# tzmhuang/OmniIsaacGymEnvs

Hardware: AMD Instinct MI355X
Metric: env-steps/s (physics+obs+reward) Humanoid 4096 envs @1/2/4/8 MI355X (higher is better)
Workload: dtype f32

## Files before the change

### include/mi_sim.h

```cpp
#ifndef MI_SIM_H
#define MI_SIM_H

#include <stdint.h>

#ifdef __cplusplus
extern "C" {
#endif

#define MI_ABI_VERSION 4

enum {
    MI_OK = 0,
    MI_E_NULL = -1,
    MI_E_SHAPE = -2,
    MI_E_HIP = -3,
    MI_E_MODEL = -4,
    MI_E_ARG = -5,
    MI_E_NODEV = -6,
    MI_E_STATE = -7
};

enum { MI_TASK_CARTPOLE = 0, MI_TASK_ANT = 1, MI_TASK_HUMANOID = 2 };

enum {
// ... 58 lines not shown
    int32_t num_obs;
    int32_t num_actions;
    float clip_actions, clip_obs;
    float max_episode_length;
    float power_scale, heading_weight, up_weight, actions_cost, energy_cost;
    float dof_vel_scale, angular_velocity_scale, contact_force_scale;
    float joints_at_limit_cost, death_cost, termination_height, alive_reward_scale;
    float task_dt;
    float target[3];
    float init_root_pos[3];
    float init_root_quat[4];
    float dof_pos_noise, dof_vel_noise;
    const float* joint_gears;
    const float* motor_effort_ratio;
    const float* init_dof_pos;
    float reset_dist, max_push_effort;
} mi_task_params;

#define MI_MAX_ROWS 128

typedef struct mi_sim mi_sim;

int mi_sim_create(const mi_model_desc* model, const mi_sim_params* params, int32_t num_envs,
                  int64_t env_id_offset, int32_t device_id, const float* env_origins ,
                  uint64_t seed, mi_sim** out);
int mi_sim_destroy(mi_sim* sim);
int mi_sim_info(const mi_sim* sim, int32_t* num_envs, int32_t* num_dof, int32_t* num_links,
                int32_t* num_sensors, float* dof_limits );

int mi_get_root_state(mi_sim* sim, float* pos , float* quat ,
                      float* vel , void* stream);
int mi_get_dof_state(mi_sim* sim, float* q , float* qd , void* stream);
int mi_get_sensor_wrench(mi_sim* sim, float* out , void* stream);
int mi_set_dof_efforts(mi_sim* sim, const float* eff , const int32_t* idx ,
                       int32_t n, void* stream);
int mi_set_dof_state(mi_sim* sim, const float* q , const float* qd ,
                     const int64_t* idx , int32_t n, void* stream);
int mi_set_root_state(mi_sim* sim, const float* pos , const float* quat ,
                      const float* vel , const int64_t* idx , int32_t n,
                      void* stream);
int mi_set_dof_state_i32(mi_sim* sim, const float* q , const float* qd ,
                         const int32_t* idx , int32_t n, void* stream);
int mi_set_root_state_i32(mi_sim* sim, const float* pos , const float* quat ,
                          const float* vel , const int32_t* idx , int32_t n,
                          void* stream);
int mi_get_link_state(mi_sim* sim, const int32_t* link_ids , const float* offsets ,
                      int32_t K, float* pos, float* quat, float* vel, void* stream);
int mi_get_link_jacobian(mi_sim* sim, const int32_t* link_ids, const float* offsets, int32_t K,
                         float* jac, void* stream);
int mi_get_dynamics(mi_sim* sim, float* M, float* cor, float* grav, void* stream);
enum { MI_MASS_ARMATURE = 0,
       MI_MASS_STEPPER  = 1 };

int mi_solve_mass(mi_sim* sim, int32_t which, const float* rhs, int32_t R, float* out, void* stream);

int mi_get_forward_dynamics(mi_sim* sim, int32_t which, const float* tau, float* acc, void* stream);

int mi_get_link_task_inertia(mi_sim* sim, int32_t which, const int32_t* link_ids, const float* offsets,
                             int32_t K, float* minv_jt, float* lam_inv, void* stream);
enum { MI_MASS_RIGID = 2 };

int mi_get_inverse_dynamics(mi_sim* sim, int32_t which, const float* acc, float* tau, float* joint_wrench,
                            void* stream);

int mi_get_link_acceleration(mi_sim* sim, const int32_t* link_ids, const float* offsets, int32_t K,
                             const float* acc, float* out, void* stream);

int mi_get_momentum(mi_sim* sim, float* com, float* mom, float* cmm, float* energy, void* stream);
int mi_sim_set_mirror(mi_sim* sim, float* pos , float* quat , float* vel ,
                      float* q , float* qd , float* sens );
int mi_get_state_mirror(mi_sim* sim, void* stream);

int mi_sim_step(mi_sim* sim, int32_t substeps, void* stream);
int mi_sim_flush(mi_sim* sim, void* stream);

int mi_task_configure(mi_sim* sim, const mi_task_params* tp);
int mi_task_pre_step(mi_sim* sim, const float* actions , int64_t* reset_buf,
                     int64_t* progress_buf, float* potentials, float* prev_potentials,
                     float* actions_out , void* stream);
int mi_task_reset_idx(mi_sim* sim, const int64_t* env_ids, int32_t n, int64_t* reset_buf,
                      int64_t* progress_buf, float* potentials, float* prev_potentials,
                      void* stream);
int mi_task_post_step(mi_sim* sim, const float* actions , float* obs ,
                      float* rew , int64_t* reset_buf, int64_t* progress_buf,
                      float* potentials, float* prev_potentials, void* stream);
int mi_task_post_kernel(const mi_sim* sim, int32_t* kernel, int32_t* grid);
int mi_task_observations(mi_sim* sim, const float* actions , float* obs ,
                         float* potentials, float* prev_potentials, void* stream);
int mi_task_metrics(mi_sim* sim, const float* actions, const float* obs, float* rew,
                    const float* potentials, const float* prev_potentials, void* stream);
int mi_task_is_done(mi_sim* sim, const float* obs, int64_t* reset_buf, const int64_t* progress_buf,
                    void* stream);
int mi_env_step(mi_sim* sim, const float* actions , int32_t substeps,
                float* obs_out , float* obs_task ,
                float* rew , int64_t* reset_buf, int64_t* progress_buf,
                float* potentials, float* prev_potentials, float* actions_out ,
                float* rew_out , int64_t* reset_out , void* stream);
int mi_sim_time_launches(mi_sim* sim, int32_t every, int32_t capacity);
int mi_sim_launch_times(mi_sim* sim, float* ms_out, int32_t max_out, int32_t* n_out);

enum { MI_DR_OP_ADDITIVE = 0, MI_DR_OP_SCALING = 1 };
enum { MI_DR_DIST_GAUSSIAN = 0, MI_DR_DIST_UNIFORM = 1, MI_DR_DIST_LOGUNIFORM = 2 };
typedef struct mi_dr_noise {
    int32_t enabled;
    int32_t operation;
    int32_t distribution;
    int32_t frequency_interval;
    float params[2];
} mi_dr_noise;
typedef struct mi_dr_params {
    mi_dr_noise obs_on_reset, obs_on_interval, act_on_reset, act_on_interval;
} mi_dr_params;
int mi_task_set_dr(mi_sim* sim, const mi_dr_params* dr );
int mi_dr_apply_actions(mi_sim* sim, float* actions , const int64_t* reset_buf, void* stream);
int mi_dr_apply_observations(mi_sim* sim, float* obs , const int64_t* reset_buf,
                             void* stream);
int mi_get_dr_state(mi_sim* sim, uint32_t* out );

enum { MI_ENVP_GRAVITY = 0,
       MI_ENVP_FRICTION = 1,
       MI_ENVP_DAMPING = 2,
       MI_ENVP_ARMATURE = 3    };
int mi_set_env_params(mi_sim* sim, int32_t attr, const float* values ,
                      const int64_t* idx , int32_t n, void* stream);
int mi_get_env_params(mi_sim* sim, int32_t attr, float* out , void* stream);
int mi_sim_clear_env_params(mi_sim* sim);

enum { MI_DR_OP_DIRECT = 2 };
typedef struct mi_dr_phys_sched {
    int32_t enabled;
    int32_t operation;
    int32_t distribution;
    int32_t frequency_interval;
    const float* p0;
    const float* p1;
} mi_dr_phys_sched;
typedef struct mi_dr_phys_params {
    mi_dr_phys_sched on_reset[4], on_interval[4];
    int32_t min_frequency;
} mi_dr_phys_params;
int mi_sim_set_phys_dr(mi_sim* sim, const mi_dr_phys_params* dr );
int mi_dr_phys_step(mi_sim* sim, const int64_t* reset_buf , void* stream);
int mi_get_phys_dr_state(mi_sim* sim, uint32_t* out );

int mi_fill_uniform(mi_sim* sim, float* out , int32_t cols, uint64_t seed,
                    uint64_t step, float lo, float hi, void* stream);
int mi_get_reset_count(mi_sim* sim, uint32_t* out );
int mi_set_reset_count(mi_sim* sim, const uint32_t* in );
int mi_sim_pair_load(mi_sim* sim, int32_t* out , const int32_t* in ,
                     int32_t pairing);
int mi_sim_nan_count(mi_sim* sim, int64_t* count);
int mi_sim_kernel_path(const mi_sim* sim, int32_t* path, int32_t* topology, int32_t* lds_bytes);
int mi_sim_w_rows_lds(const mi_sim* sim, int32_t* rows);
int mi_abi_version(void);
const char* mi_build_id(void);
const char* mi_last_error(void);

#ifdef __cplusplus
}
#endif
#endif
```

### omniisaacgymenvs_amd/csrc/mi_pair.hpp

```cpp
#pragma once
#include "mi_wave.hpp"

#ifndef MI_PAIR_SOLVE_PD
#define MI_PAIR_SOLVE_PD 3
#endif
#ifndef MI_PRIO_C1
#define MI_PRIO_C1 12
#endif
#ifndef MI_PRIO_C2
#define MI_PRIO_C2 18
#endif
#ifndef MI_PRIO_C3
#define MI_PRIO_C3 27
#endif

namespace mi {

MI_D float pbc(float v, int k) {
    const float a = readlane(v, k), b = readlane(v, k + 32);
    return (pair_l64() & 32) ? b : a;
}
template <int K>
MI_D float pbcc(float v) {
    static_assert(K >= 0 && K < 32, "lane of the half");
// ... 17 lines not shown
        const int c = __popc((m >> b) & ((1u << w) - 1u));
        if (j >= c) { j -= c; b += w; }
    }
    return b;
}
MI_D unsigned low_bits(unsigned m, int k) {
    return k >= __popc(m) ? m : (m & ((1u << nth_bit(m, k)) - 1u));
}
MI_D int pmax(int v) { return max(__builtin_amdgcn_readlane(v, 0), __builtin_amdgcn_readlane(v, 32)); }
MI_D float psum(float v) { return pbc(half_sums(v), 31); }

template <class T>
MI_D float ct_ltdl_pair(int lane, float (&Mc)[T::nvc]) {
    float dvec = 1.0f;
    sfor_down<0, T::nv>([&](auto K) {
        constexpr int k = K;
        const int ln = lane_here(lane);
        const float inv = __builtin_amdgcn_rcpf(pbcc<k>(Mc[k]));
        const float t = Mc[k] * inv;
        sfor<T::dof.anc_start[k], T::dof.anc_start[k + 1]>([&](auto A) {
            constexpr int ii = T::dof.anc[A];
            Mc[ii] -= pbcc<ii>(t) * Mc[k];
        });
        Mc[k] = t;
        dvec = ln == k ? inv : dvec;
    });
    return dvec;
}

#ifndef MI_PAIR_WIDE_PD
#define MI_PAIR_WIDE_PD 16
#endif
#ifndef MI_PAIR_WIDE_AREG
#define MI_PAIR_WIDE_AREG 28
#endif
constexpr int kWideScratchRows = 64 - MI_PAIR_WIDE_AREG;
#ifndef MI_PAIR_WIDE_AP
#define MI_PAIR_WIDE_AP 8
#endif
#ifndef MI_PAIR_LIM_NEAR
#define MI_PAIR_LIM_NEAR 0.05f
#endif
#ifndef MI_PAIR_LIM_SPEC_MIN_D
#define MI_PAIR_LIM_SPEC_MIN_D 16
#endif
#ifndef MI_PAIR_JREUSE_MAXNV
#define MI_PAIR_JREUSE_MAXNV 16
#endif
typedef float pv2 __attribute__((ext_vector_type(2)));
template <int NV, int NVC>
MI_D float pk_jdot(const float (&J)[NVC], const float* u) {
    float v = 0.0f;
    sfor<0, NV>([&](auto C) { v += J[C] * u[C]; });
    return v;
}

template <class TP>
MI_D void pair_jrow(const MC& mc, const WaveTabs& t, const float* sm, int r, int nr,
                    float (&J)[TP::nvc]) {
    const float lk = sm[t.s_rl + r];
    float f[6] = {0.0f, 0.0f, 0.0f, 0.0f, 0.0f, 0.0f};
    unsigned msk = 0u, msk2 = 0u;
    float sg = 0.0f;
    int kdof = -1;
    if (lk >= 0.0f) {
        msk = mc.mask((int)lk);
        const float l2 = TP::kSelf ? sm[t.s_cl2 + r / 3] : -1.0f;
        msk2 = l2 >= 0.0f ? mc.mask((int)l2) : 0u;
        contact_row_f<TP::kSelf>(sm, t, r, f);
    } else {
        kdof = (int)(-lk - 1.0f);
        sg = sm[t.s_lsg + kdof - nr];
    }
    const float* Ss = sm + t.s_S;
    sdof_loop<TP, MI_PAIR_SDOF_PD, false, sdof_first_loaded(TP::nr)>(Ss, nullptr, [&](auto C, const float (&sv)[6], float) {
        constexpr int c = C;
        const float v = sdot<TP, c>(sv, f);
        const bool ia = (msk >> c) & 1u, ib = (msk2 >> c) & 1u;
        float xc = (ia ? v : 0.0f) - (ib ? v : 0.0f);
        asm volatile("" : "+v"(xc));
        J[c] = kdof >= 0 ? (kdof == c ? sg : 0.0f) : xc;
    });
}

typedef const float __attribute__((address_space(3)))* lds_cf;
MI_D lds_cf lds_ptr(const float* p) { return (lds_cf)p; }
typedef float pv4 __attribute__((ext_vector_type(4)));
typedef const pv4 __attribute__((address_space(3)))* lds_cf4;
MI_D int pw_idx(int r, int c, int nv) { return (r & ~3) * nv + 4 * c + (r & 3); }
MI_D size_t pair_sidx(int r, int c) { return (size_t)(r & ~3) * WNV + 4 * c + (r & 3); }
typedef const float __attribute__((address_space(1)))* glb_cf;
typedef float __attribute__((address_space(1)))* glb_f;
typedef const pv4 __attribute__((address_space(1)))* glb_cf4;
MI_D glb_cf glb_ptr(const float* p) { return (glb_cf)p; }
MI_D glb_f glb_ptr(float* p) { return (glb_f)p; }

struct WSrc {
    lds_cf W;
    glb_cf gW;
    int nl;
};
MI_D WSrc make_wsrc(const WaveTabs& t, const float* sm, glb_cf gW) {
    WSrc w;
    w.W = lds_ptr(sm + t.s_W);
    int nl = t.w_rows_lds;
    asm volatile("" : "+s"(nl));
    w.nl = nl;
    w.gW = gW;
    return w;
}

template <class TP, int PD, bool kLds>
MI_D void pair_dgroup_w(const WSrc& ws, int g0, int n, const float (&Jr)[TP::nvc], float (&a)[4]) {
    constexpr int NV = TP::nv, NB = PD + 1;
    pv2 a01 = {0.0f, 0.0f}, a23 = {0.0f, 0.0f};
    auto acc = [&](auto C, const pv4& w) {
        const pv2 j = {Jr[C], Jr[C]};
        a01 = __builtin_elementwise_fma(j, w.xy, a01);
        a23 = __builtin_elementwise_fma(j, w.zw, a23);
    };
    if (kLds || g0 + 3 < ws.nl) {
        const lds_cf4 W = (lds_cf4)(ws.W + g0 * NV);
        pv4 wb[NB];
        sfor<0, (PD < NV ? PD : NV)>([&](auto C) { wb[C % NB] = W[C]; });
        sfor<0, NV>([&](auto C) {
            constexpr int c = C;
            if constexpr (c + PD < NV) wb[(c + PD) % NB] = W[c + PD];
            acc(C, wb[c % NB]);
        });
    } else {
        const glb_cf4 W = (glb_cf4)(ws.gW + (size_t)g0 * WNV);
        pv4 wb[NB];
        sfor<0, (PD < NV ? PD : NV)>([&](auto C) { wb[C % NB] = W[C]; });
        sfor<0, NV>([&](auto C) {
            constexpr int c = C;
            if constexpr (c + PD < NV) wb[(c + PD) % NB] = W[c + PD];
            acc(C, wb[c % NB]);
        });
    }
    const float a0 = a01.x, a1 = a01.y, a2 = a23.x, a3 = a23.y;
    a[0] = g0 < n ? a0 : 0.0f;
    a[1] = g0 + 1 < n ? a1 : 0.0f;
    a[2] = g0 + 2 < n ? a2 : 0.0f;
    a[3] = g0 + 3 < n ? a3 : 0.0f;
}
template <bool kLds>
MI_D void pair_wcol_w(const WSrc& ws, int g0, int kc, int nv, float (&wq)[4]) {
    const pv4 w = (kLds || g0 + 3 < ws.nl) ? ((lds_cf4)(ws.W + g0 * nv))[kc]
                                           : ((glb_cf4)(ws.gW + (size_t)g0 * WNV))[kc];
    wq[0] = w.x; wq[1] = w.y; wq[2] = w.z; wq[3] = w.w;
}


template <class TP>
MI_D void pair_artic_substep(const DevModel& m, const WaveTabs& t, const DevState& st,
                             const SimP& p, int i, int wv_, const float* mcb, float* sm, float* gW_,
                             bool load_state, bool store_state, int& prio, int& load,
                             const float* ep = nullptr) {
    const glb_f gW = glb_ptr(gW_);
    static_assert(TP::kCT && TP::nv <= 32, "paired kernel: compiled topology, nv <= 32");
    const int lane = pair_l64() & 31;
    const int L = m.L, D = m.D, nv = m.nv, nr = m.nr;
    const float dt = p.dt;
    float* us = sm + t.s_us;
    float* rhs = sm + t.s_r;
    float* Mx = sm + t.s_M;
    float* Ss = sm + t.s_S;
    const MC mc = make_mc(t, mcb, L);

    STAMP_BEGIN();
    if (load_state) {
        if (lane < 3) sm[t.s_rp + lane] = st.root_pos[sx(st, lane, i)];
        if (lane < 4) sm[t.s_rp + 4 + lane] = st.root_quat[sx(st, lane, i)];
        if (lane < nr) us[lane] = st.root_vel[sx(st, lane, i)];
        else if (lane < nv) us[lane] = st.qd[sx(st, lane - nr, i)];
        if (lane < D) sm[t.s_q + lane] = st.q[sx(st, lane, i)];
    }
    if (nr && lane < 6) {
        float s[6] = {0, 0, 0, 0, 0, 0};
        if (lane < 3) s[3 + lane] = 1.0f; else s[lane - 3] = 1.0f;
#pragma unroll
        for (int c = 0; c < 6; ++c) Ss[6 * lane + c] = s[c];
    }
    wave_sync();
    STAMP(0);
    for (int l = 1 + lane; l < L; l += 32) wave_link_local(mc, t, sm, l);
    wave_sync();
    for (int l = lane; l < L; l += 32) wave_link_forward<TP::kEnvP>(mc, nr, t, sm, l, p, ep);
    wave_sync();
    STAMP(1);
    float* aux = sm + t.s_X;
    {
        const pv4* recs = reinterpret_cast<const pv4*>(sm + t.s_F);
        for (int l = lane; l < L; l += 32) {
            pv4 a0 = recs[4 * l], a1 = recs[4 * l + 1], a2 = recs[4 * l + 2], a3 = recs[4 * l + 3];
            for (int di = mc.desc_start(l); di < mc.desc_start(l + 1); ++di) {
                const int d = mc.desc(di);
                a0 += recs[4 * d];
                a1 += recs[4 * d + 1];
                a2 += recs[4 * d + 2];
                a3 += recs[4 * d + 3];
            }
            pv4* o = reinterpret_cast<pv4*>(aux) + 4 * l;
            o[0] = a0; o[1] = a1; o[2] = a2; o[3] = a3;
        }
    }
    wave_sync();
    STAMP(2);
    phase_p3_bias_crba<Grp32, TP>(lane, i, D, nv, nr, dt, us, rhs, Mx, Ss, mc, t, st, aux, ep);
    wave_sync();
    STAMP(3);
    float Mc[TP::nvc];
    ct_load_columns<TP>(Mx, lane, Mc);
    const float dvec = ct_ltdl_pair<TP>(lane, Mc);
    STAMP(5);
    {
        const int dj = lane < nr ? lane : __builtin_popcount(mc.mask(lane < nv ? lane - nr + 1 : 0)) - 1;
        ct_publish_factor<TP>(lane, dj, Mc, dvec, sm + t.s_L);
    }
    STAMP(4);
    int ncon = 0;
    {
        const float rpz = sm[t.s_rp + 2];
        for (int c0 = 0; c0 < t.npts; c0 += 32) {
            const int c = c0 + lane;
            bool act = false;
            float pc[3] = {0, 0, 0}, bn = 0.0f;
            int l = 0;
            if (c < t.npts) {
                l = (int)mc.pf(MP_LINK, c);
                const float pl[3] = {mc.pf(MP_X, c), mc.pf(MP_X + 1, c), mc.pf(MP_X + 2, c)};
                float R[9], x[3];
#pragma unroll
                for (int q = 0; q < 9; ++q) R[q] = sm[t.s_R + 9 * l + q];
                m3_vec(R, pl, x);
#pragma unroll
                for (int q = 0; q < 3; ++q) x[q] += sm[t.s_o + 3 * l + q];
                const float rr = mc.pf(MP_RAD, c);
                const float gap = rpz + x[2] - rr;
                act = gap < p.contact_offset;
                pc[0] = x[0]; pc[1] = x[1]; pc[2] = x[2] - rr;
                const float d = gap - p.rest_offset;
                bn = p.tgs ? d : row_bias(p, d, dt, true);
            }
            const unsigned mask = hballot(act);
            if (act) {
                const int ci = ncon + __popc(mask & lanemask_lt(lane));
#pragma unroll
                for (int q = 0; q < 3; ++q) sm[t.s_cp + 3 * ci + q] = pc[q];
                sm[t.s_cl + ci] = (float)l;
                sm[t.s_cl2 + ci] = -1.0f;
#pragma unroll
                for (int tt = 0; tt < 3; ++tt) {
                    const int r = 3 * ci + tt;
                    sm[t.s_rl + r] = (float)l;
                    sm[t.s_rb + r] = tt == 0 ? bn : 0.0f;
                }
            }
            ncon += __popc(mask);
        }
    }
    if constexpr (TP::kSelf) {
        if (t.self_on) {
            float* seg = sm + t.s_seg;
            float* bnd = seg + 8 * t.ngeoms;
            const float* geo = mcb + t.mc_geo;
            const int2* gpr = reinterpret_cast<const int2*>(t.g_pairs);
            int2 gpf[5];
#pragma unroll
            for (int q = 0; q < 5; ++q) {
                const int pi = 32 * q + lane;
                gpf[q] = pi < t.npairs ? gpr[pi] : make_int2(0, 0);
            }
            for (int g = lane; g < t.ngeoms; g += 32) {
                const float* A = geo + 8 * g;
                const int l = (int)A[0];
                float R[9], a0[3], a1[3];
#pragma unroll
                for (int q = 0; q < 9; ++q) R[q] = sm[t.s_R + 9 * l + q];
                m3_vec(R, A + 1, a0); m3_vec(R, A + 4, a1);
#pragma unroll
                for (int q = 0; q < 3; ++q) {
                    seg[8 * g + q] = a0[q] + sm[t.s_o + 3 * l + q];
                    seg[8 * g + 3 + q] = a1[q] + sm[t.s_o + 3 * l + q];
                }
                seg[8 * g + 6] = A[7];
                seg[8 * g + 7] = (float)l;
                float e2 = 0.0f;
#pragma unroll
                for (int q = 0; q < 3; ++q) {
                    bnd[4 * g + q] = sm[t.s_o + 3 * l + q] + 0.5f * (a0[q] + a1[q]);
                    e2 += (a1[q] - a0[q]) * (a1[q] - a0[q]);
                }
                bnd[4 * g + 3] = 0.5f * sqrtf(e2) + A[7];
            }
            wave_sync();
            int* surv = reinterpret_cast<int*>(sm + t.s_surv);
            int nsv = 0;
            const float slack = p.contact_offset + 1e-3f;
            auto broad = [&](int pb, int2 gpq, bool pref) {
                const int pi = pb + lane;
                bool keep = false;
                int2 gp = make_int2(0, 0);
                if (pi < t.npairs) {
                    gp = pref ? gpq : gpr[pi];
                    const float4 A = *reinterpret_cast<const float4*>(bnd + 4 * gp.x);
                    const float4 B = *reinterpret_cast<const float4*>(bnd + 4 * gp.y);
                    const float cx = A.x - B.x, cy = A.y - B.y, cz = A.z - B.z;
                    const float reach = A.w + B.w + slack;
                    keep = cx * cx + cy * cy + cz * cz < reach * reach;
                }
                const unsigned mask = hballot(keep);
                if (keep) surv[nsv + __popc(mask & lanemask_lt(lane))] = gp.x | (gp.y << 16);
                nsv += __popc(mask);
            };
            sfor<0, 5>([&](auto Q) { if (32 * (int)Q < t.npairs) broad(32 * (int)Q, gpf[Q], true); });
            for (int pb = 160; pb < t.npairs; pb += 32) broad(pb, make_int2(0, 0), false);
            wave_sync();
            int budget = (MI_MAX_ROWS - 3 * ncon - t.nlimc) / 3;
            const int nsv_max = pmax(nsv);
            for (int sb = 0; sb < nsv_max; sb += 32) {
                const int sidx = sb + lane;
                bool act = false;
                float pc[3], n[3], bn = 0.0f;
                int la = 0, lb = 0;
                if (sidx < nsv && budget > 0) {
                    const int pk = surv[sidx];
                    const float* A = seg + 8 * (pk & 0xffff);
                    const float* B = seg + 8 * (pk >> 16);
                    la = (int)A[7]; lb = (int)B[7];
                    const float gap = mi_pair_contact(A, A + 3, A[6], B, B + 3, B[6], pc, n);
                    act = gap < p.contact_offset;
                    const float d = gap - p.rest_offset;
                    bn = p.tgs ? d : row_bias(p, d, dt, true);
                }
                const unsigned mask = hballot(act);
                const int rank = __popc(mask & lanemask_lt(lane));
                if (act && rank < budget) {
                    const int ci = ncon + rank;
#pragma unroll
                    for (int q = 0; q < 3; ++q) { sm[t.s_cp + 3 * ci + q] = pc[q]; sm[t.s_cn + 3 * ci + q] = n[q]; }
                    sm[t.s_cl + ci] = (float)la;
                    sm[t.s_cl2 + ci] = (float)lb;
#pragma unroll
                    for (int tt = 0; tt < 3; ++tt) {
                        const int r = 3 * ci + tt;
                        sm[t.s_rl + r] = (float)la;
                        sm[t.s_rb + r] = tt == 0 ? bn : 0.0f;
                    }
                }
                const int took = budget > 0 ? min(__popc(mask), budget) : 0;
                ncon += took;
                budget -= took;
            }
        }
    }
    const int nc = 3 * ncon;
    {
        const int cr = pmax(nc);
// ... 849 lines not shown
```

### omniisaacgymenvs_amd/csrc/mi_sim.hip

```cpp
#include <hip/hip_runtime.h>
#include <hip/hip_ext.h>

#include <cmath>
#include <cstdarg>
#include <cstdio>
#include <cstring>
#include <string>
#include <vector>
#include <algorithm>

#include "mi_artic.hpp"
#include "mi_device.hpp"
#include "mi_task.hpp"
#include "mi_wave.hpp"
#include "mi_pair.hpp"
#include "mi_link.hpp"
#include "mi_dyn.hpp"
#include "mi_msolve.hpp"
#include "mi_idyn.hpp"

using namespace mi;

static thread_local std::string g_err;

// ... 858 lines not shown
    __shared__ float tile[MI_GATHER_MAXC * (MI_GATHER_TILE + 1)];
    for (int c = 0; c < C; ++c)
        if ((int)threadIdx.x < ne) tile[c * (MI_GATHER_TILE + 1) + threadIdx.x] = g.src[(size_t)c * fs + e0 + threadIdx.x];
    __syncthreads();
    for (int t = threadIdx.x; t < tot; t += blockDim.x) {
        const int e = t / C, c = t - e * C;
        out[t] = tile[c * (MI_GATHER_TILE + 1) + e];
    }
}
template <typename IDX>
__global__ __launch_bounds__(256) void k_rows_to_soa_multi(GFields fs3, int n, const IDX* __restrict__ idx,
                                                          int N, int fs, int es) {
    const GField g = fs3.f[blockIdx.y];
    const int64_t t = (int64_t)blockIdx.x * blockDim.x + threadIdx.x;
    if (t >= (int64_t)n * g.C) return;
    const int r = (int)(t / g.C), c = (int)(t - (int64_t)r * g.C);
    const int64_t i = idx ? (int64_t)idx[r] : r;
    if (i < 0 || i >= N) return;
    const_cast<float*>(g.dst)[(size_t)c * fs + (size_t)i * es] = g.src[t];
}
static inline dim3 gather_grid(int N) { return dim3((N + MI_GATHER_TILE - 1) / MI_GATHER_TILE); }
static inline dim3 scatter_grid(int n, int C) { return dim3((unsigned)(((int64_t)n * C + 255) / 256)); }

__global__ void k_init_state(DevState st, int D) {
    const int i = blockIdx.x * blockDim.x + threadIdx.x;
    if (i >= st.N) return;
    const int N = st.N;
    for (int k = 0; k < 3; ++k) st.root_pos[sx(st, k, i)] = st.origins[(size_t)k * N + i];
    st.root_quat[sx(st, 0, i)] = 1.0f;
}

__global__ void k_fill_uniform(int N, int64_t off, float* out, int cols, uint64_t seed,
                               uint64_t step, float lo, float hi) {
    const int i = blockIdx.x * blockDim.x + threadIdx.x;
    if (i >= N) return;
    const uint64_t gid = (uint64_t)(off + i);
    const float w = hi - lo;
    float u[4];
    for (int c = 0; c < cols; ++c) {
        if ((c & 3) == 0) uniform4(seed, gid, (uint32_t)step, (uint32_t)(c >> 2), 1, u);
        out[(size_t)i * cols + c] = w * u[c & 3] + lo;
    }
}

static inline int envp_base(int attr, int D) { return attr == MI_ENVP_GRAVITY ? 0 : attr == MI_ENVP_FRICTION ? 3 : attr == MI_ENVP_DAMPING ? 4 : 4 + D; }
static inline int envp_dim(int attr, int D) { return attr == MI_ENVP_GRAVITY ? 3 : attr == MI_ENVP_FRICTION ? 1 : D; }

__global__ __launch_bounds__(256) void k_envp_fill(float* __restrict__ envp, int stride, int recw,
                                                   const float* __restrict__ nominal, int N) {
    const int64_t t = (int64_t)blockIdx.x * blockDim.x + threadIdx.x;
    if (t >= (int64_t)N * stride) return;
    const int k = (int)(t % stride);
    envp[t] = k < recw ? nominal[k] : 0.0f;
}
__global__ __launch_bounds__(256) void k_envp_set(float* __restrict__ envp, int stride, int base, int dim,
                                                  const float* __restrict__ values,
                                                  const int64_t* __restrict__ idx, int n, int N) {
    const int64_t t = (int64_t)blockIdx.x * blockDim.x + threadIdx.x;
    if (t >= (int64_t)n * dim) return;
    const int r = (int)(t / dim), c = (int)(t - (int64_t)r * dim);
    const int64_t i = idx ? idx[r] : (int64_t)r;
    if (i < 0 || i >= N) return;
    envp[(size_t)i * stride + base + c] = values[t];
}
__global__ __launch_bounds__(256) void k_envp_get(const float* __restrict__ envp, int stride, int base, int dim,
                                                  const float* __restrict__ nominal, float* __restrict__ out,
                                                  int N) {
    const int64_t t = (int64_t)blockIdx.x * blockDim.x + threadIdx.x;
    if (t >= (int64_t)N * dim) return;
    const int i = (int)(t / dim), c = (int)(t - (int64_t)i * dim);
    out[t] = envp ? envp[(size_t)i * stride + base + c] : nominal[base + c];
}

struct PhysDR {
    int min_frequency, freq, any_interval, pad;
    int r_on[4], r_op[4], r_dist[4], i_on[4], i_op[4], i_dist[4];
};
__global__ __launch_bounds__(256) void k_dr_phys_step(int N, int64_t off, uint64_t seed, int D,
                                                      const PhysDR* __restrict__ d,
                                                      const float* __restrict__ prm,
                                                      const float* __restrict__ nominal,
                                                      uint32_t* __restrict__ ps, float* __restrict__ envp,
                                                      int stride, const int64_t* __restrict__ reset_buf) {
    const int i = blockIdx.x * blockDim.x + threadIdx.x;
    if (i >= N) return;
    const size_t n = (size_t)N;
    const mi_dr_phys_env e = mi_dr_phys_begin(ps[i], ps[n + i], ps[2 * n + i], ps[3 * n + i],
                                              reset_buf[i] != 0, d->min_frequency, d->any_interval, d->freq);
    ps[i] = e.since; ps[n + i] = e.counter; ps[2 * n + i] = e.epoch; ps[3 * n + i] = e.draws;
    if (!(e.reset || e.fire)) return;
    const uint64_t gid = (uint64_t)(off + i);
    const int recw = 4 + 2 * D;
    float* rec = envp + (size_t)i * stride;
    for (int a = 0; a < MI_DR_PHYS_ATTRS; ++a) {
        const int r_on = d->r_on[a], i_on = d->i_on[a];
        if (!((e.reset && r_on) || (e.fire && i_on))) continue;
        const int base = a == 0 ? 0 : a == 1 ? 3 : a == 2 ? 4 : 4 + D;
        const int dim = a == 0 ? 3 : a == 1 ? 1 : D;
        float ur[4] = {0.0f, 0.0f, 0.0f, 0.0f}, ui[4] = {0.0f, 0.0f, 0.0f, 0.0f};
        for (int c = 0; c < dim; ++c) {
            if ((c & 1) == 0) {
                if (r_on && e.epoch) uniform4(seed, gid, e.epoch, (uint32_t)(c >> 1), MI_DR_STREAM_PHYS_RESET(a), ur);
                if (i_on && e.draws) uniform4(seed, gid, e.draws, (uint32_t)(c >> 1), MI_DR_STREAM_PHYS_INTERVAL(a), ui);
            }
            const int k = base + c;
            rec[k] = mi_dr_phys_value(nominal[k], c, r_on, d->r_op[a], d->r_dist[a], prm[k], prm[recw + k],
                                      e.epoch, ur, i_on, d->i_op[a], d->i_dist[a], prm[2 * recw + k],
                                      prm[3 * recw + k], e.draws, ui);
        }
    }
}

extern "C" {

int mi_abi_version(void) { return MI_ABI_VERSION; }
#ifndef MI_BUILD_ID
#define MI_BUILD_ID "unknown"
#endif
const char* mi_build_id(void) {
    static const char id[] = MI_BUILD_ID;
    return (sizeof(id) > 12 && id[0] == 'M' && id[11] == ':') ? id + 12 : id;
}

#ifdef MI_STAMPS
int mi_debug_stamps(unsigned long long* out, int n) {
    if (!out || n <= 0 || n > 32) return MI_E_ARG;
    HIP_TRY(hipDeviceSynchronize());
    std::vector<unsigned long long> all((size_t)MI_STAMP_SLOTS * 32);
    HIP_TRY(hipMemcpyFromSymbol(all.data(), HIP_SYMBOL(g_phase), all.size() * sizeof(unsigned long long)));
    for (int k = 0; k < n; ++k) {
        unsigned long long acc = 0;
        for (size_t b = 0; b < (size_t)MI_STAMP_SLOTS; ++b) acc += all[b * 32 + k];
        out[k] = acc;
    }
    std::fill(all.begin(), all.end(), 0ull);
    HIP_TRY(hipMemcpyToSymbol(HIP_SYMBOL(g_phase), all.data(), all.size() * sizeof(unsigned long long)));
    return MI_OK;
}
#endif
#ifdef MI_STAMPS
int mi_debug_stamps_raw(unsigned long long* out, int slots) {
    if (!out || slots <= 0 || slots > MI_STAMP_SLOTS) return MI_E_ARG;
    HIP_TRY(hipDeviceSynchronize());
    std::vector<unsigned long long> all((size_t)MI_STAMP_SLOTS * 32);
    HIP_TRY(hipMemcpyFromSymbol(all.data(), HIP_SYMBOL(g_phase), all.size() * sizeof(unsigned long long)));
    std::copy(all.begin(), all.begin() + (size_t)slots * 32, out);
    std::fill(all.begin(), all.end(), 0ull);
    HIP_TRY(hipMemcpyToSymbol(HIP_SYMBOL(g_phase), all.data(), all.size() * sizeof(unsigned long long)));
    return MI_OK;
}
#endif
const char* mi_last_error(void) { return g_err.c_str(); }

struct CreateCtx {
    const mi_model_desc* md;
    const mi_sim_params* prm;
    bool self_on = false;
    std::vector<int> dof_parent, dof_link, pt_geom, pt_end;
    std::vector<int> chain_start, chain_list, desc_start, desc_list, anc_start;
    std::vector<unsigned long long> link_mask;
};
#define UP(field, src, cnt) if (int rc = upload(s, src, (size_t)(cnt), &m.field)) return rc
#define UPW(field, vec) if (int rc = upload(s, vec.data(), vec.size(), &t.field)) return rc
#define AL(field, T, cnt) if (int rc = dev_alloc(s, &p, sizeof(T) * (size_t)(cnt))) return rc; st.field = (T*)p

static int create_validate(const mi_model_desc* md, int32_t N) {
    if (N <= 0) return fail(MI_E_SHAPE, "num_envs must be > 0 (got %d)", N);
    const int L = md->num_links;
    if (L < 1 || L - 1 > MI_MAXA) return fail(MI_E_MODEL, "num_links %d out of range [1,%d]", L, MI_MAXA + 1);
    if (md->dyn_kind != MI_DYN_ARTICULATION && md->dyn_kind != MI_DYN_CARTPOLE)
        return fail(MI_E_ARG, "bad dyn_kind %d", md->dyn_kind);
    if (md->dyn_kind == MI_DYN_CARTPOLE && L != 3)
        return fail(MI_E_MODEL, "cart-pole dynamics needs exactly 2 joints");
    if (!md->parent || !md->jtype || !md->axis || !md->pos || !md->quat || !md->mass || !md->com ||
        !md->inertia || !md->lower || !md->upper || !md->damping || !md->armature)
        return fail(MI_E_NULL, "model arrays must not be null");
    if (md->num_geoms < 0 || md->num_sensors < 0 || md->num_pairs < 0)
        return fail(MI_E_MODEL, "negative counts");
    if (md->num_geoms && (!md->geom_link || !md->geom_type || !md->geom_p0 || !md->geom_p1 || !md->geom_radius))
        return fail(MI_E_NULL, "geom arrays must not be null");
    if (md->num_sensors && (!md->sensor_link || !md->sensor_pos))
        return fail(MI_E_NULL, "sensor arrays must not be null");
    for (int l = 1; l < L; ++l)
        if (md->parent[l] < 0 || md->parent[l] >= l)
            return fail(MI_E_MODEL, "parent[%d]=%d must be in [0,%d)", l, md->parent[l], l);
    for (int g = 0; g < md->num_geoms; ++g)
        if (md->geom_link[g] < 0 || md->geom_link[g] >= L) return fail(MI_E_MODEL, "geom_link[%d] out of range", g);
    for (int s = 0; s < md->num_sensors; ++s)
        if (md->sensor_link[s] < 0 || md->sensor_link[s] >= L) return fail(MI_E_MODEL, "sensor_link[%d] out of range", s);
    if (md->num_pairs && !md->pairs) return fail(MI_E_NULL, "pairs must not be null");
    for (int q = 0; q < 2 * md->num_pairs; ++q)
        if (md->pairs[q] < 0 || md->pairs[q] >= md->num_geoms)
            return fail(MI_E_MODEL, "pairs[%d]=%d is not a geom index", q, md->pairs[q]);
    return MI_OK;
}

static int create_model(mi_sim* s, CreateCtx& cx) {
    const mi_model_desc* md = cx.md;
    const int L = md->num_links;
    DevModel& m = s->dm;
    m.dyn = md->dyn_kind;
    m.root_free = md->root_free ? 1 : 0;
    m.L = L;
    m.D = L - 1;
    m.nr = m.root_free ? 6 : 0;
    m.nv = m.nr + m.D;
    m.G = md->num_geoms;
    m.S = md->num_sensors;
    if (m.nv > MI_MAXNV) return fail(MI_E_MODEL, "too many dofs");
    std::vector<int>&dof_parent = cx.dof_parent, &dof_link = cx.dof_link, &pt_geom = cx.pt_geom, &pt_end = cx.pt_end;
    dof_parent.assign(m.nv > 0 ? m.nv : 1, 0);
    dof_link.assign(m.nv > 0 ? m.nv : 1, 0);
    for (int k = 0; k < m.nr; ++k) { dof_parent[k] = k - 1; dof_link[k] = 0; }
    for (int l = 1; l < L; ++l) {
        const int k = m.nr + l - 1, P = md->parent[l];
        dof_parent[k] = P == 0 ? m.nr - 1 : m.nr + P - 1;
        dof_link[k] = l;
    }
    for (int g = 0; g < m.G; ++g) {
        pt_geom.push_back(g); pt_end.push_back(0);
        if (md->geom_type[g] == MI_GEOM_CAPSULE) { pt_geom.push_back(g); pt_end.push_back(1); }
    }
    m.npts = (int)pt_geom.size();
    const bool self_on = cx.self_on = cx.prm->enable_self_collisions && md->num_pairs > 0 &&
                         md->dyn_kind == MI_DYN_ARTICULATION;
    m.max_rows = 3 * m.npts + m.D;
    if (m.max_rows > MI_MAX_ROWS)
        return fail(MI_E_MODEL, "%d contact points + %d joints exceed the %d-row budget",
                            m.npts, m.D, MI_MAX_ROWS);
    if (self_on) m.max_rows = std::min(MI_MAX_ROWS, 3 * (m.npts + md->num_pairs) + m.D);
    UP(parent, md->parent, L); UP(jtype, md->jtype, L); UP(axis, md->axis, 3 * L);
    UP(pos, md->pos, 3 * L); UP(quat, md->quat, 4 * L); UP(mass, md->mass, L);
    UP(com, md->com, 3 * L); UP(inertia, md->inertia, 6 * L); UP(lower, md->lower, L);
    UP(upper, md->upper, L); UP(damping, md->damping, L); UP(armature, md->armature, L);
    UP(dof_parent, dof_parent.data(), dof_parent.size()); UP(dof_link, dof_link.data(), dof_link.size());
    UP(geom_link, md->geom_link, m.G); UP(geom_p0, md->geom_p0, 3 * m.G);
    UP(geom_p1, md->geom_p1, 3 * m.G); UP(geom_radius, md->geom_radius, m.G);
    UP(pt_geom, pt_geom.data(), pt_geom.size()); UP(pt_end, pt_end.data(), pt_end.size());
    UP(sensor_link, md->sensor_link, m.S); UP(sensor_pos, md->sensor_pos, 3 * m.S);
    m.cart_mass = md->cart_mass; m.pole_mass = md->pole_mass; m.pole_com = md->pole_com;
    m.pole_inertia = md->pole_inertia; m.cart_damping = md->cart_damping;
    m.pole_damping = md->pole_damping;
    int o = 0;
    if (m.dyn == MI_DYN_ARTICULATION) {
        const int nv = m.nv, R = m.max_rows;
        m.o_R = o; o += 9 * L;
        m.o_o = o; o += 3 * L;
        m.o_aw = o;
        m.o_Ic = o; o += 10 * L;
        m.o_S = o; o += 6 * nv;
        m.o_V = o; o += 6 * L;
        m.o_A = o; o += 6 * L;
        m.o_F = o; o += 6 * L;
        m.o_M = o; o += nv * nv;
        m.o_u = o; o += nv;
        m.o_r = o; o += nv;
        m.o_Jr = o; o += R * nv;
        m.o_W = o; o += R * nv;
        m.o_b = o; o += R;
        m.o_lam = o; o += R;
        m.o_Ad = o; o += R;
        m.o_rk = o; o += R;
        m.o_ds = o; o += R;
        m.o_cp = o; o += 3 * m.npts;
        m.o_cl = o; o += m.npts;
    }
    m.slots = o;
    s->lower.assign(md->lower, md->lower + L);
    s->upper.assign(md->upper, md->upper + L);
    return MI_OK;
}

static int create_path(mi_sim* s, const CreateCtx& cx) {
    const DevModel& m = s->dm;
    const int L = m.L;
    const bool self_on = cx.self_on;
    {
        const char* path = getenv("MI_SIM_PATH");
        const bool want_thread = path && std::string(path) == "thread";
        s->wave = m.dyn == MI_DYN_ARTICULATION && !want_thread && m.nv <= WNV && m.npts <= 64 &&
                  m.max_rows <= 128 && L <= 64 && m.max_rows >= 6 * m.S + 3 * m.D;
        if (self_on && !s->wave)
            return fail(MI_E_MODEL, "self-collision needs the wavefront-per-env path "
                                            "(one-lane-per-env path %s)", want_thread ? "forced by MI_SIM_PATH" : "selected");
    }
    if (s->wave) {
        const char* tsel = getenv("MI_SIM_TOPO");
        s->topo = (tsel && std::string(tsel) == "runtime") ? 0 : match_topology(cx.md, self_on);
    }
    return MI_OK;
}

static int create_tree_tables(mi_sim* s, CreateCtx& cx) {
    const mi_model_desc* md = cx.md;
    const DevModel& m = s->dm;
    WaveTabs& t = s->wt;
    const int L = m.L;
    const std::vector<int>& dof_parent = cx.dof_parent;
    std::vector<int> depth(L, 0);
    int maxd = 0;
    for (int l = 1; l < L; ++l) { depth[l] = depth[md->parent[l]] + 1; maxd = std::max(maxd, depth[l]); }
    t.nlev = maxd + 1;
    std::vector<int> lev_start(t.nlev + 1, 0), lev_links;
    for (int d = 0; d < t.nlev; ++d) {
        lev_start[d] = (int)lev_links.size();
        for (int l = 0; l < L; ++l) if (depth[l] == d) lev_links.push_back(l);
// ... 1475 lines not shown
```

### omniisaacgymenvs_amd/csrc/mi_topo.hpp

```cpp
#pragma once
#include <type_traits>

namespace mi {

template <int B, int E, class F>
__device__ __forceinline__ void sfor(F&& f) {
    if constexpr (B < E) {
        f(std::integral_constant<int, B>{});
        sfor<B + 1, E>(f);
    }
}
template <int B, int E, class F>
__device__ __forceinline__ void sfor_down(F&& f) {
    if constexpr (B < E) {
        f(std::integral_constant<int, E - 1>{});
        sfor_down<B, E - 1>(f);
    }
}

template <int NV>
struct DofTree {
    int parent[NV > 0 ? NV : 1];
    int anc_start[NV + 1];
    int anc[NV * NV > 0 ? NV * NV : 1];
    unsigned anc_mask[NV > 0 ? NV : 1];
    unsigned col_rows[32];
    int anc_total;
    int lrow[NV + 1];
};

template <int L, int NR>
constexpr DofTree<NR + L - 1> make_dof_tree(const int (&link_parent)[L]) {
    constexpr int NV = NR + L - 1;
    DofTree<NV> t{};
    for (int k = 0; k < NR; ++k) t.parent[k] = k - 1;
    for (int l = 1; l < L; ++l) {
        const int p = link_parent[l];
        t.parent[NR + l - 1] = p == 0 ? NR - 1 : NR + p - 1;
    }
    int n = 0;
    for (int k = 0; k < NV; ++k) {
        t.anc_start[k] = n;
        t.anc_mask[k] = 0u;
        for (int j = t.parent[k]; j >= 0; j = t.parent[j]) {
            t.anc[n++] = j;
            t.anc_mask[k] |= 1u << j;
        }
    }
    t.anc_start[NV] = n;
    t.anc_total = n;
    for (int j = 0; j < 32; ++j) t.col_rows[j] = 0u;
    for (int k = 0; k < NV; ++k)
        for (int j = 0; j < NV; ++j)
            if (j == k || ((t.anc_mask[k] >> j) & 1u)) t.col_rows[j] |= 1u << k;
    int o = 0;
    for (int k = 0; k < NV; ++k) {
        t.lrow[k] = o;
        o += (t.anc_start[k + 1] - t.anc_start[k] + 3) & ~3;
    }
    t.lrow[NV] = o;
    return t;
}

struct TopoRuntime {
    static constexpr bool kCT = false;
    static constexpr bool kSelf = true;
    static constexpr int id = 0;
    static constexpr int nvc = 1;
    static constexpr int kLamRows = 0;
    static constexpr int kWaves = 2;
    static constexpr bool kTgs = false;
    static constexpr bool kEnvP = false;
};

template <class R>
struct TopoCT {
    static constexpr bool kCT = true;
    static constexpr bool kSelf = R::self;
    static constexpr int id = R::id;
    static constexpr int L = R::L, nr = R::nr, D = R::L - 1, nv = R::nr + R::L - 1, nvc = nv;
    static constexpr DofTree<nv> dof = make_dof_tree<R::L, R::nr>(R::link_parent);
    static constexpr int kLamRows = R::self ? 32 : 24;
#ifdef MI_WAVES_ALL
    static constexpr int kWaves = MI_WAVES_ALL;
#else
    static constexpr int kWaves = R::self ? 2 : 4;
#endif
    static_assert(nv <= 32, "compile-time topology supports nv <= 32 (anc_mask is 32-bit)");
    static constexpr bool kTgs = false;
    static constexpr bool kEnvP = false;
};

template <class T>
struct Tgs : T {
    static constexpr bool kTgs = true;
};

template <class T>
struct EnvP : T {
    static constexpr bool kEnvP = true;
};
constexpr int kEnvpFriction = 3, kEnvpDamping = 4;

}
```

### omniisaacgymenvs_amd/native.py

```python
from __future__ import annotations

import ctypes as C
import os
from typing import Optional

import numpy as np

_HERE = os.path.dirname(os.path.abspath(__file__))
LIB_PATH = os.environ.get("MI_SIM_LIB", os.path.join(_HERE, "libmi_sim.so"))

MI_OK = 0
MI_TASK_CARTPOLE, MI_TASK_ANT, MI_TASK_HUMANOID = 0, 1, 2
MI_DYN_ARTICULATION, MI_DYN_CARTPOLE = 0, 1
MI_SOLVER_PGS, MI_SOLVER_TGS = 0, 1
MI_JOINT_HINGE, MI_JOINT_SLIDE = 0, 1
MI_GEOM_SPHERE, MI_GEOM_CAPSULE = 0, 1

_f32p = C.POINTER(C.c_float)
_i32p = C.POINTER(C.c_int32)
_i64p = C.POINTER(C.c_int64)


class MiModelDesc(C.Structure):
    _fields_ = [
        ("dyn_kind", C.c_int32), ("root_free", C.c_int32), ("num_links", C.c_int32),
        ("num_geoms", C.c_int32), ("num_sensors", C.c_int32), ("num_pairs", C.c_int32),
        ("parent", _i32p), ("jtype", _i32p), ("axis", _f32p), ("pos", _f32p), ("quat", _f32p),
        ("mass", _f32p), ("com", _f32p), ("inertia", _f32p), ("lower", _f32p), ("upper", _f32p),
        ("damping", _f32p), ("armature", _f32p), ("geom_link", _i32p), ("geom_type", _i32p),
        ("geom_p0", _f32p), ("geom_p1", _f32p), ("geom_radius", _f32p), ("sensor_link", _i32p),
        ("sensor_pos", _f32p), ("pairs", _i32p),
        ("cart_mass", C.c_float), ("pole_mass", C.c_float), ("pole_com", C.c_float),
        ("pole_inertia", C.c_float), ("cart_damping", C.c_float), ("pole_damping", C.c_float),
    ]


class MiSimParams(C.Structure):
    _fields_ = [
        ("dt", C.c_float), ("gravity", C.c_float * 3), ("solver_iterations", C.c_int32),
        ("contact_offset", C.c_float), ("rest_offset", C.c_float), ("friction", C.c_float),
        ("max_depenetration_velocity", C.c_float), ("erp", C.c_float),
        ("enable_self_collisions", C.c_int32), ("max_angular_velocity", C.c_float),
        ("angular_damping", C.c_float), ("solver_type", C.c_int32), ("velocity_iterations", C.c_int32),
    ]


class MiTaskParams(C.Structure):
    _fields_ = [
        ("task_kind", C.c_int32), ("num_obs", C.c_int32), ("num_actions", C.c_int32),
        ("clip_actions", C.c_float), ("clip_obs", C.c_float), ("max_episode_length", C.c_float),
        ("power_scale", C.c_float), ("heading_weight", C.c_float), ("up_weight", C.c_float),
        ("actions_cost", C.c_float), ("energy_cost", C.c_float), ("dof_vel_scale", C.c_float),
        ("angular_velocity_scale", C.c_float), ("contact_force_scale", C.c_float),
        ("joints_at_limit_cost", C.c_float), ("death_cost", C.c_float),
        ("termination_height", C.c_float), ("alive_reward_scale", C.c_float),
        ("task_dt", C.c_float), ("target", C.c_float * 3), ("init_root_pos", C.c_float * 3),
        ("init_root_quat", C.c_float * 4), ("dof_pos_noise", C.c_float),
        ("dof_vel_noise", C.c_float), ("joint_gears", _f32p), ("motor_effort_ratio", _f32p),
        ("init_dof_pos", _f32p), ("reset_dist", C.c_float), ("max_push_effort", C.c_float),
    ]


MI_DR_OP_ADDITIVE, MI_DR_OP_SCALING = 0, 1
MI_DR_DIST_GAUSSIAN, MI_DR_DIST_UNIFORM, MI_DR_DIST_LOGUNIFORM = 0, 1, 2


class MiDrNoise(C.Structure):
    _fields_ = [("enabled", C.c_int32), ("operation", C.c_int32), ("distribution", C.c_int32),
                ("frequency_interval", C.c_int32), ("params", C.c_float * 2)]


class MiDrParams(C.Structure):
    _fields_ = [("obs_on_reset", MiDrNoise), ("obs_on_interval", MiDrNoise),
                ("act_on_reset", MiDrNoise), ("act_on_interval", MiDrNoise)]


MI_DR_OP_DIRECT = 2
MI_ENVP_GRAVITY, MI_ENVP_FRICTION, MI_ENVP_DAMPING, MI_ENVP_ARMATURE = 0, 1, 2, 3
MI_MASS_ARMATURE, MI_MASS_STEPPER = 0, 1
MI_MASS_RIGID = 2


class MiDrPhysSched(C.Structure):
    _fields_ = [("enabled", C.c_int32), ("operation", C.c_int32), ("distribution", C.c_int32),
                ("frequency_interval", C.c_int32), ("p0", _f32p), ("p1", _f32p)]


class MiDrPhysParams(C.Structure):
    _fields_ = [("on_reset", MiDrPhysSched * 4), ("on_interval", MiDrPhysSched * 4),
                ("min_frequency", C.c_int32)]


def fptr(a: Optional[np.ndarray]):
    return None if a is None else a.ctypes.data_as(_f32p)


def iptr(a: Optional[np.ndarray]):
    return None if a is None else a.ctypes.data_as(_i32p)


class NativeUnavailable(RuntimeError):
    """libmi_sim.so could not be used: not built, failed to load, or no GPU."""


_LIB = None

_SIGS = {
    "mi_sim_create": (C.c_int, [C.POINTER(MiModelDesc), C.POINTER(MiSimParams), C.c_int32,
                                C.c_int64, C.c_int32, C.c_void_p, C.c_uint64, C.POINTER(C.c_void_p)]),
    "mi_sim_destroy": (C.c_int, [C.c_void_p]),
    "mi_sim_info": (C.c_int, [C.c_void_p, _i32p, _i32p, _i32p, _i32p, C.c_void_p]),
    "mi_get_root_state": (C.c_int, [C.c_void_p] + [C.c_void_p] * 4),
    "mi_get_dof_state": (C.c_int, [C.c_void_p] + [C.c_void_p] * 3),
    "mi_get_sensor_wrench": (C.c_int, [C.c_void_p, C.c_void_p, C.c_void_p]),
    "mi_get_link_state": (C.c_int, [C.c_void_p, _i32p, _f32p, C.c_int32, C.c_void_p, C.c_void_p, C.c_void_p,
                                    C.c_void_p]),
    "mi_get_link_jacobian": (C.c_int, [C.c_void_p, _i32p, _f32p, C.c_int32, C.c_void_p, C.c_void_p]),
    "mi_get_dynamics": (C.c_int, [C.c_void_p] + [C.c_void_p] * 4),
    "mi_solve_mass": (C.c_int, [C.c_void_p, C.c_int32, C.c_void_p, C.c_int32, C.c_void_p, C.c_void_p]),
    "mi_get_forward_dynamics": (C.c_int, [C.c_void_p, C.c_int32, C.c_void_p, C.c_void_p, C.c_void_p]),
    "mi_get_link_task_inertia": (C.c_int, [C.c_void_p, C.c_int32, _i32p, _f32p, C.c_int32, C.c_void_p, C.c_void_p,
                                           C.c_void_p]),
    "mi_get_inverse_dynamics": (C.c_int, [C.c_void_p, C.c_int32, C.c_void_p, C.c_void_p, C.c_void_p, C.c_void_p]),
    "mi_get_link_acceleration": (C.c_int, [C.c_void_p, _i32p, _f32p, C.c_int32, C.c_void_p, C.c_void_p, C.c_void_p]),
    "mi_get_momentum": (C.c_int, [C.c_void_p] + [C.c_void_p] * 5),
    "mi_set_dof_efforts": (C.c_int, [C.c_void_p, C.c_void_p, C.c_void_p, C.c_int32, C.c_void_p]),
    "mi_set_dof_state": (C.c_int, [C.c_void_p, C.c_void_p, C.c_void_p, C.c_void_p, C.c_int32,
                                   C.c_void_p]),
    "mi_set_root_state": (C.c_int, [C.c_void_p, C.c_void_p, C.c_void_p, C.c_void_p, C.c_void_p,
                                    C.c_int32, C.c_void_p]),
    "mi_set_dof_state_i32": (C.c_int, [C.c_void_p, C.c_void_p, C.c_void_p, C.c_void_p, C.c_int32,
                                       C.c_void_p]),
    "mi_set_root_state_i32": (C.c_int, [C.c_void_p, C.c_void_p, C.c_void_p, C.c_void_p, C.c_void_p,
                                        C.c_int32, C.c_void_p]),
    "mi_sim_set_mirror": (C.c_int, [C.c_void_p] + [C.c_void_p] * 6),
    "mi_get_state_mirror": (C.c_int, [C.c_void_p, C.c_void_p]),
    "mi_sim_step": (C.c_int, [C.c_void_p, C.c_int32, C.c_void_p]),
    "mi_sim_flush": (C.c_int, [C.c_void_p, C.c_void_p]),
    "mi_task_configure": (C.c_int, [C.c_void_p, C.POINTER(MiTaskParams)]),
    "mi_task_pre_step": (C.c_int, [C.c_void_p] + [C.c_void_p] * 7),
    "mi_task_reset_idx": (C.c_int, [C.c_void_p, C.c_void_p, C.c_int32] + [C.c_void_p] * 5),
    "mi_task_post_step": (C.c_int, [C.c_void_p] + [C.c_void_p] * 8),
    "mi_task_post_kernel": (C.c_int, [C.c_void_p, _i32p, _i32p]),
    "mi_task_observations": (C.c_int, [C.c_void_p] + [C.c_void_p] * 5),
    "mi_task_metrics": (C.c_int, [C.c_void_p] + [C.c_void_p] * 6),
    "mi_task_is_done": (C.c_int, [C.c_void_p] + [C.c_void_p] * 4),
    "mi_env_step": (C.c_int, [C.c_void_p, C.c_void_p, C.c_int32] + [C.c_void_p] * 11),
    "mi_sim_time_launches": (C.c_int, [C.c_void_p, C.c_int32, C.c_int32]),
    "mi_sim_launch_times": (C.c_int, [C.c_void_p, C.c_void_p, C.c_int32, _i32p]),
    "mi_task_set_dr": (C.c_int, [C.c_void_p, C.POINTER(MiDrParams)]),
    "mi_dr_apply_actions": (C.c_int, [C.c_void_p, C.c_void_p, C.c_void_p, C.c_void_p]),
    "mi_dr_apply_observations": (C.c_int, [C.c_void_p, C.c_void_p, C.c_void_p, C.c_void_p]),
    "mi_get_dr_state": (C.c_int, [C.c_void_p, C.c_void_p]),
    "mi_set_env_params": (C.c_int, [C.c_void_p, C.c_int32, C.c_void_p, C.c_void_p, C.c_int32, C.c_void_p]),
    "mi_get_env_params": (C.c_int, [C.c_void_p, C.c_int32, C.c_void_p, C.c_void_p]),
    "mi_sim_clear_env_params": (C.c_int, [C.c_void_p]),
    "mi_sim_set_phys_dr": (C.c_int, [C.c_void_p, C.POINTER(MiDrPhysParams)]),
    "mi_dr_phys_step": (C.c_int, [C.c_void_p, C.c_void_p, C.c_void_p]),
    "mi_get_phys_dr_state": (C.c_int, [C.c_void_p, C.c_void_p]),
    "mi_fill_uniform": (C.c_int, [C.c_void_p, C.c_void_p, C.c_int32, C.c_uint64, C.c_uint64,
                                  C.c_float, C.c_float, C.c_void_p]),
    "mi_get_reset_count": (C.c_int, [C.c_void_p, C.c_void_p]),
    "mi_set_reset_count": (C.c_int, [C.c_void_p, C.c_void_p]),
    "mi_sim_pair_load": (C.c_int, [C.c_void_p, C.c_void_p, C.c_void_p, C.c_int32]),
    "mi_sim_nan_count": (C.c_int, [C.c_void_p, _i64p]),
    "mi_sim_kernel_path": (C.c_int, [C.c_void_p, _i32p, _i32p, _i32p]),
    "mi_sim_w_rows_lds": (C.c_int, [C.c_void_p, _i32p]),
    "mi_abi_version": (C.c_int, []),
    "mi_build_id": (C.c_char_p, []),
    "mi_last_error": (C.c_char_p, []),
}

EXPORTED_SYMBOLS = tuple(_SIGS)


def load_library(path: str = LIB_PATH) -> C.CDLL:
    if not os.path.exists(path):
        raise NativeUnavailable(
            f"{path} is missing: build it with `python -c 'import __graft_entry__ as g; g.build()'`")
    try:
        lib = C.CDLL(path)
    except OSError as e:
        raise NativeUnavailable(f"failed to load {path}: {e}") from e
    lenient = "MI_SIM_LIB" in os.environ and path == LIB_PATH
    for name, (res, args) in _SIGS.items():
        try:
            fn = getattr(lib, name)
        except AttributeError:
            if lenient and name == "mi_build_id":
                continue
            raise
        fn.restype = res
        fn.argtypes = args
    return lib


def lib() -> C.CDLL:
    global _LIB
    if _LIB is None:
        _LIB = load_library()
    return _LIB


def check(rc: int, what: str = "") -> None:
    if rc != MI_OK:
        msg = lib().mi_last_error()
        raise RuntimeError(f"{what or 'mi_sim'} failed ({rc}): {msg.decode() if msg else ''}")


def ptr(t) -> Optional[int]:
    if t is None:
        return None
    return t.data_ptr()
```

Before: 40.80 million.

## Spread composite-inertia accumulation across 4 lanes per link with descendant-sorted order

```diff
diff --git a/include/mi_sim.h b/include/mi_sim.h
--- a/include/mi_sim.h
+++ b/include/mi_sim.h
@@ -234,6 +234,8 @@
 int mi_sim_nan_count(mi_sim* sim, int64_t* count);
 int mi_sim_kernel_path(const mi_sim* sim, int32_t* path, int32_t* topology, int32_t* lds_bytes);
 int mi_sim_w_rows_lds(const mi_sim* sim, int32_t* rows);
+int mi_p2_item_table(const int32_t* link_parent, int32_t L, int32_t lanes, int32_t* items, int32_t cap,
+                     int32_t* passes);
 int mi_abi_version(void);
 const char* mi_build_id(void);
 const char* mi_last_error(void);
diff --git a/omniisaacgymenvs_amd/csrc/mi_pair.hpp b/omniisaacgymenvs_amd/csrc/mi_pair.hpp
--- a/omniisaacgymenvs_amd/csrc/mi_pair.hpp
+++ b/omniisaacgymenvs_amd/csrc/mi_pair.hpp
@@ -193,6 +193,52 @@
 }
 
 
+constexpr int kP2Batch = 4;
+template <class TP>
+constexpr bool p2_decode_is_table() {
+    for (int p = 0; p < p2_passes(TP::L, 32); ++p)
+        for (int ln = 0; ln < 32; ++ln) {
+            const bool has = 8 * p + (ln >> 2) < TP::L;
+            const int it = has ? 4 * p2_unpack(TP::p2.pk[p], ln >> 2) + (ln & 3) : -1;
+            if (it != p2_item(TP::p2.pk, TP::L, 32, p, ln)) return false;
+        }
+    return true;
+}
+template <class TP>
+MI_D void pair_p2_composites(int lane, const MC& mc, const WaveTabs& t, const float* sm, float* aux) {
+    static_assert(p2_decode_is_table<TP>(), "P2 item decode");
+    constexpr int B = kP2Batch;
+    const pv4* recs = reinterpret_cast<const pv4*>(sm + t.s_F);
+    pv4* out = reinterpret_cast<pv4*>(aux);
+    const int* dl = mc.bi + t.mc_dsl;
+    const int ln = lane_here(lane) & 31;
+    const int slot = ln & 3, sub = ln >> 2;
+    sfor<0, p2_passes(TP::L, 32)>([&](auto P) {
+        constexpr int p = P;
+        const int l = p2_unpack(TP::p2.pk[p], sub);
+        if (8 * p + sub < TP::L) {
+            const int ds = mc.desc_start(l), de = mc.desc_start(l + 1);
+            pv4 a = recs[4 * l + slot];
+            int id[B];
+            if (ds < de) {
+#pragma unroll
+                for (int k = 0; k < B; ++k) id[k] = dl[min(ds + k, de - 1)];
+            }
+            for (int di = ds; di < de; di += B) {
+                pv4 r[B];
+#pragma unroll
+                for (int k = 0; k < B; ++k) r[k] = recs[4 * id[k] + slot];
+#pragma unroll
+                for (int k = 0; k < B; ++k) id[k] = dl[min(di + B + k, de - 1)];
+#pragma unroll
+                for (int k = 0; k < B; ++k)
+                    if (di + k < de) a += r[k];
+            }
+            out[4 * l + slot] = a;
+        }
+    });
+}
+
 template <class TP>
 MI_D void pair_artic_substep(const DevModel& m, const WaveTabs& t, const DevState& st,
                              const SimP& p, int i, int wv_, const float* mcb, float* sm, float* gW_,
@@ -231,21 +277,7 @@
     wave_sync();
     STAMP(1);
     float* aux = sm + t.s_X;
-    {
-        const pv4* recs = reinterpret_cast<const pv4*>(sm + t.s_F);
-        for (int l = lane; l < L; l += 32) {
-            pv4 a0 = recs[4 * l], a1 = recs[4 * l + 1], a2 = recs[4 * l + 2], a3 = recs[4 * l + 3];
-            for (int di = mc.desc_start(l); di < mc.desc_start(l + 1); ++di) {
-                const int d = mc.desc(di);
-                a0 += recs[4 * d];
-                a1 += recs[4 * d + 1];
-                a2 += recs[4 * d + 2];
-                a3 += recs[4 * d + 3];
-            }
-            pv4* o = reinterpret_cast<pv4*>(aux) + 4 * l;
-            o[0] = a0; o[1] = a1; o[2] = a2; o[3] = a3;
-        }
-    }
+    pair_p2_composites<TP>(lane, mc, t, sm, aux);
     wave_sync();
     STAMP(2);
     phase_p3_bias_crba<Grp32, TP>(lane, i, D, nv, nr, dt, us, rhs, Mx, Ss, mc, t, st, aux, ep);
diff --git a/omniisaacgymenvs_amd/csrc/mi_sim.hip b/omniisaacgymenvs_amd/csrc/mi_sim.hip
--- a/omniisaacgymenvs_amd/csrc/mi_sim.hip
+++ b/omniisaacgymenvs_amd/csrc/mi_sim.hip
@@ -1034,6 +1034,28 @@
 #endif
 const char* mi_last_error(void) { return g_err.c_str(); }
 
+int mi_p2_item_table(const int32_t* link_parent, int32_t L, int32_t lanes, int32_t* items, int32_t cap,
+                     int32_t* passes) {
+    if (!link_parent || !passes) return fail(MI_E_ARG, "mi_p2_item_table: NULL argument");
+    if (L < 1 || L > kP2MaxLinks || (lanes != 32 && lanes != 64))
+        return fail(MI_E_ARG, "mi_p2_item_table: L in 1..64, lanes 32 or 64");
+    if (link_parent[0] != -1) return fail(MI_E_ARG, "mi_p2_item_table: link 0 is the root (parent -1)");
+    for (int l = 1; l < L; ++l)
+        if (link_parent[l] < 0 || link_parent[l] >= l)
+            return fail(MI_E_ARG, "mi_p2_item_table: parents precede their children");
+    const int np = p2_passes(L, lanes);
+    *passes = np;
+    if (!items) return MI_OK;
+    if (cap < np * lanes) return fail(MI_E_ARG, "mi_p2_item_table: items holds fewer than passes * lanes entries");
+    int order[kP2MaxLinks], ndesc[kP2MaxLinks];
+    unsigned long long pk[kP2MaxLinks / 8];
+    p2_link_order(link_parent, L, order, ndesc);
+    p2_pack(order, L, pk);
+    for (int p = 0; p < np; ++p)
+        for (int ln = 0; ln < lanes; ++ln) items[p * lanes + ln] = p2_item(pk, L, lanes, p, ln);
+    return MI_OK;
+}
+
 struct CreateCtx {
     const mi_model_desc* md;
     const mi_sim_params* prm;
diff --git a/omniisaacgymenvs_amd/csrc/mi_topo.hpp b/omniisaacgymenvs_amd/csrc/mi_topo.hpp
--- a/omniisaacgymenvs_amd/csrc/mi_topo.hpp
+++ b/omniisaacgymenvs_amd/csrc/mi_topo.hpp
@@ -62,6 +62,44 @@
     return t;
 }
 
+constexpr int kP2MaxLinks = 64;
+constexpr void p2_link_order(const int* link_parent, int L, int* order, int* ndesc) {
+    for (int l = 0; l < L; ++l) ndesc[l] = 0;
+    for (int c = 1; c < L; ++c)
+        for (int x = link_parent[c]; x >= 0; x = link_parent[x]) ++ndesc[x];
+    for (int l = 0; l < L; ++l) {
+        int at = l;
+        for (; at > 0 && ndesc[order[at - 1]] < ndesc[l]; --at) order[at] = order[at - 1];
+        order[at] = l;
+    }
+}
+constexpr void p2_pack(const int* order, int L, unsigned long long* pk) {
+    for (int w = 0; w < (L + 7) / 8; ++w) pk[w] = 0ull;
+    for (int r = 0; r < L; ++r) pk[r >> 3] |= (unsigned long long)order[r] << (6 * (r & 7));
+}
+constexpr int p2_unpack(unsigned long long word, int sub) { return (int)(word >> (6 * sub)) & 63; }
+constexpr int p2_item(const unsigned long long* pk, int L, int W, int pass, int lane) {
+    const int rank = pass * (W / 4) + (lane >> 2);
+    return rank < L ? 4 * p2_unpack(pk[rank >> 3], rank & 7) + (lane & 3) : -1;
+}
+constexpr int p2_passes(int L, int W) { return (4 * L + W - 1) / W; }
+
+template <int L>
+struct P2Items {
+    static_assert(L <= kP2MaxLinks, "link ids are packed in 6 bits");
+    static constexpr int kWords = (L + 7) / 8;
+    int order[L];
+    int ndesc[L];
+    unsigned long long pk[kWords];
+};
+template <int L>
+constexpr P2Items<L> make_p2_items(const int (&link_parent)[L]) {
+    P2Items<L> t{};
+    p2_link_order(link_parent, L, t.order, t.ndesc);
+    p2_pack(t.order, L, t.pk);
+    return t;
+}
+
 struct TopoRuntime {
     static constexpr bool kCT = false;
     static constexpr bool kSelf = true;
@@ -80,6 +118,7 @@
     static constexpr int id = R::id;
     static constexpr int L = R::L, nr = R::nr, D = R::L - 1, nv = R::nr + R::L - 1, nvc = nv;
     static constexpr DofTree<nv> dof = make_dof_tree<R::L, R::nr>(R::link_parent);
+    static constexpr P2Items<R::L> p2 = make_p2_items<R::L>(R::link_parent);
     static constexpr int kLamRows = R::self ? 32 : 24;
 #ifdef MI_WAVES_ALL
     static constexpr int kWaves = MI_WAVES_ALL;
diff --git a/omniisaacgymenvs_amd/native.py b/omniisaacgymenvs_amd/native.py
--- a/omniisaacgymenvs_amd/native.py
+++ b/omniisaacgymenvs_amd/native.py
@@ -166,6 +166,7 @@
     "mi_sim_nan_count": (C.c_int, [C.c_void_p, _i64p]),
     "mi_sim_kernel_path": (C.c_int, [C.c_void_p, _i32p, _i32p, _i32p]),
     "mi_sim_w_rows_lds": (C.c_int, [C.c_void_p, _i32p]),
+    "mi_p2_item_table": (C.c_int, [_i32p, C.c_int32, C.c_int32, _i32p, C.c_int32, _i32p]),
     "mi_abi_version": (C.c_int, []),
     "mi_build_id": (C.c_char_p, []),
     "mi_last_error": (C.c_char_p, []),
@@ -187,7 +188,7 @@
         try:
             fn = getattr(lib, name)
         except AttributeError:
-            if lenient and name == "mi_build_id":
+            if lenient and name in ("mi_build_id", "mi_p2_item_table"):
                 continue
             raise
         fn.restype = res
```

New measurement: 41.48 million (median of 6 runs). +1.7%, better.
